# kcleal/pywfa

Measured on AMD Instinct MI355X. Metric: pairwise alignments/sec, higher is better.
Workload: dtype int16x2 offsets (reads <= 512 bp), int32 results; 1 GPU; C2: 10000000 x 150bp pairs/GPU, 2% error, gap-affine 0/4/6/2, end-to-end, scope=score, 2-bit reads resident in HBM; pairs_per_gpu=10000000, read_length=150, parallelism=pairs sharded over 1 GPU(s), no collective

## Files before the change

### pywfa_amd/csrc/wfa_lane.hpp

```cpp
#pragma once
#include "wfa_rtc_compat.hpp"
#include "wfa_common.hpp"
#include "wfa_hip.h"
#ifndef __HIPCC_RTC__
#include "wfa_rtc.hpp"
#endif

namespace wfa {

typedef short lane_s2 __attribute__((ext_vector_type(2)));
typedef unsigned short lane_u2 __attribute__((ext_vector_type(2)));

#define WFA_LANE_NULL16 (-16384)
#define WFA_LANE_NULL2 0xC000C000u
#ifndef WFA_LANE_DEBUG_COUNTERS
#define WFA_LANE_DEBUG_COUNTERS 0
#endif
#ifndef WFA_LANE_REGION_MARKS
#define WFA_LANE_REGION_MARKS 0
#endif
#if WFA_LANE_REGION_MARKS
#define WFA_LANE_MARK(name) asm volatile("; WFA_MARK " name ::: "memory")
#else
#define WFA_LANE_MARK(name)
#endif
#define WFA_LANE_COUNT(i) do { if (WFA_LANE_DEBUG_COUNTERS && !FULL && a.hist) { if (lane == 0) atomicAdd(reinterpret_cast<unsigned long long*>(a.hist) + (i), 1ull); } } while (0)

__device__ __forceinline__ uint32_t lane_ffbl(uint32_t x) {
  uint32_t r;
  asm("v_ffbl_b32 %0, %1" : "=v"(r) : "v"(x));
  return r;
}
__device__ __forceinline__ uint32_t pk_max(uint32_t a, uint32_t b) {
  lane_s2 r = __builtin_elementwise_max(__builtin_bit_cast(lane_s2, a), __builtin_bit_cast(lane_s2, b));
  return __builtin_bit_cast(uint32_t, r);
}
__device__ __forceinline__ uint32_t pk_min(uint32_t a, uint32_t b) {
  lane_s2 r = __builtin_elementwise_min(__builtin_bit_cast(lane_s2, a), __builtin_bit_cast(lane_s2, b));
  return __builtin_bit_cast(uint32_t, r);
}
__device__ __forceinline__ uint32_t pk_sub(uint32_t a, uint32_t b) {
  lane_s2 r = __builtin_bit_cast(lane_s2, a) - __builtin_bit_cast(lane_s2, b);
  return __builtin_bit_cast(uint32_t, r);
}
__device__ __forceinline__ uint32_t pk_add(uint32_t a, uint32_t b) {
  lane_s2 r = __builtin_bit_cast(lane_s2, a) + __builtin_bit_cast(lane_s2, b);
  return __builtin_bit_cast(uint32_t, r);
}
__device__ __forceinline__ uint32_t pk_clamp(uint32_t nm, uint32_t lim) {
#ifndef __HIPCC_RTC__
  uint32_t d, m, r;
  asm("v_pk_sub_i16 %0, %1, %2" : "=v"(d) : "v"(lim), "v"(nm));
  asm("v_pk_ashrrev_i16 %0, 15, %1 op_sel_hi:[0,1]" : "=v"(m) : "v"(d));
  asm("v_bfi_b32 %0, %1, %2, %3" : "=v"(r) : "v"(m), "s"(WFA_LANE_NULL2), "v"(nm));
  return r;
#else
  lane_s2 d = __builtin_bit_cast(lane_s2, lim) - __builtin_bit_cast(lane_s2, nm);
  d = d >> (short)15;
  const uint32_t m = __builtin_bit_cast(uint32_t, d);
  return (nm & ~m) | (WFA_LANE_NULL2 & m);
#endif
}

#ifndef WFA_LANE_WAVES_PER_EU
#define WFA_LANE_WAVES_PER_EU 0
#endif
#if WFA_LANE_WAVES_PER_EU > 0
#define WFA_LANE_OCCUPANCY __attribute__((amdgpu_waves_per_eu(WFA_LANE_WAVES_PER_EU, WFA_LANE_WAVES_PER_EU)))
#else
#define WFA_LANE_OCCUPANCY
#endif

template <int OE, int E>
struct LaneFull { static constexpr int NREC = 2 * (OE - E) + E * 17 + 1; };

template <int X, int OE, int E, bool FULL, bool HEUR = false, int LIN = 0, int NRP = 8>
__global__ void __launch_bounds__(64) WFA_LANE_OCCUPANCY
wfa_lane_kernel(const FastArgs a, const int slot_words_seq, const int refill_arg) {
  static_assert(!(FULL && HEUR), "the general form is score only");
  static_assert(NRP == 8 || (HEUR && NRP == 16) || (NRP == 4 && !FULL && !HEUR && LIN == 0),
                "the wider band exists in the general form only, the narrow one in the plain score-only form only");
  const int refill_min = refill_arg & 0xff;
  constexpr int NR = NRP, W = 2 * NR, H = NR;
  constexpr int DM = (X > OE) ? X : OE;
  constexpr int NEVER = 0x7fffffff;
  constexpr bool ENTRY = !FULL && !HEUR && LIN == 0;
  constexpr int K = ENTRY ? OE : 0, NCH = (OE + X - 1) / X;
  constexpr int NREC = LaneFull<OE, E>::NREC;
  extern __shared__ uint32_t lds[];
  const int slot_words = slot_words_seq;
  const int lane = threadIdx.x;
  uint32_t nwork = __builtin_amdgcn_readfirstlane(a.nwork_dev ? *a.nwork_dev : a.nwork);
  const bool dyn = !FULL && a.dyn_next != nullptr;
  bool exhausted = !dyn;
  uint32_t begin, end;
  auto grab = [&](uint32_t& b_, uint32_t& e_) -> bool {
    uint32_t nb = 0;
    if (lane == 0) nb = atomicAdd(a.dyn_next, a.dyn_chunk);
    nb = __builtin_amdgcn_readfirstlane(nb);
    if (nb >= nwork) return false;
    b_ = nb; e_ = (uint32_t)min((unsigned long long)nwork, (unsigned long long)nb + a.dyn_chunk);
    return true;
  };
  if (dyn) {
    if (!grab(begin, end)) return;
  } else {
    const uint32_t per = __builtin_amdgcn_readfirstlane((nwork + gridDim.x - 1) / gridDim.x);
    const unsigned long long begin64 = (unsigned long long)blockIdx.x * per;
    if (begin64 >= nwork) return;
    begin = (uint32_t)begin64;
    end = (uint32_t)min((unsigned long long)nwork, begin64 + per);
  }

  uint32_t pid0, pw0, ln0, pid1, pw1, ln1;
  auto load_window = [&](uint32_t wb, uint32_t& pid, uint32_t& pw, uint32_t& ln) {
    const unsigned long long idx = (unsigned long long)wb + lane;
    pid = 0u; pw = 0u; ln = 0u;
    if (idx < end) {
      pid = a.worklist ? a.worklist[a.work_begin + idx] : (uint32_t)(a.work_begin + idx);
      const WfaPairMeta m = a.meta[pid];
      pw = m.p_woff;
      ln = (m.plen > WFA_FAST_MAX_LEN || m.tlen > WFA_FAST_MAX_LEN) ? 0xffffffffu : ((uint32_t)m.plen | ((uint32_t)m.tlen << 16));
    }
  };
  uint32_t wbase = begin, next_i = begin;
  load_window(wbase, pid0, pw0, ln0);
  load_window(wbase + 64u, pid1, pw1, ln1);

  const int pbase = (4 + lane * slot_words) * 16;
  uint32_t cur[NR], lim[NR], Mh[DM][NR], Ih[E][NR], Dh[E][NR];
  uint32_t thr[HEUR ? NR : 1];
#pragma unroll
  for (int r = 0; r < NR; ++r) {
    cur[r] = WFA_LANE_NULL2; lim[r] = WFA_LANE_NULL2;
    if (HEUR) thr[r] = 0x3fff3fffu;
#pragma unroll
    for (int d = 0; d < DM; ++d) Mh[d][r] = WFA_LANE_NULL2;
#pragma unroll
    for (int d = 0; d < E; ++d) { Ih[d][r] = WFA_LANE_NULL2; Dh[d][r] = WFA_LANE_NULL2; }
  }
  int kb0 = pbase, tb = pbase;
  int jt = 0;
  uint32_t tend = 0xffffu;
  int s0 = 0, deadline = NEVER;
  uint32_t my_lb2 = 0, my_tl2 = 0;
  int steps_wait = 0, my_dinit = 0;
  bool edge_live = false;
  uint32_t mypid = 0;
  unsigned long long idle = ~0ull;
  int gstep = 0;
  uint32_t myslot = 0;
  uint2* const wave_codes = FULL ? a.codes + (unsigned long long)blockIdx.x * (unsigned long long)a.codes_cap * 64ull : nullptr;
  bool codes_full = false;
  __shared__ uint32_t rejq[128];
  int nrej = 0;
  auto rej_flush = [&]() {
    if (nrej == 0) return;
    uint32_t slot = 0;
    if (lane == 0) slot = atomicAdd(a.fb_count, (uint32_t)nrej);
    slot = __builtin_amdgcn_readfirstlane(slot);
    if (lane < nrej) a.fb_list[slot + lane] = rejq[lane];
    if (lane + 64 < nrej) a.fb_list[slot + 64 + lane] = rejq[64 + lane];
    nrej = 0;
  };

  while (true) {
    WFA_LANE_MARK("looptop_begin");
    const int nidle = __builtin_popcountll(idle);
    if (!exhausted && next_i >= end && (nidle >= refill_min || idle == ~0ull)) {
      if (grab(begin, end)) { wbase = begin; next_i = begin; load_window(wbase, pid0, pw0, ln0); load_window(wbase + 64u, pid1, pw1, ln1); }
      else exhausted = true;
    }
    if (next_i < end && (nidle >= refill_min || idle == ~0ull)) {
      WFA_LANE_MARK("refill_begin");
      WFA_LANE_COUNT(1);
      const bool is_idle = __builtin_amdgcn_inverse_ballot_w64(idle);
      const uint32_t rank = __builtin_amdgcn_mbcnt_hi((uint32_t)(idle >> 32), __builtin_amdgcn_mbcnt_lo((uint32_t)idle, 0u));
      const uint32_t navail = end - next_i;
      const bool take = is_idle && rank < navail;
      const uint32_t src = next_i + rank - wbase;
      const int sl = (int)(src & 63u);
      const uint32_t a_pid = __shfl(pid0, sl, 64), a_pw = __shfl(pw0, sl, 64), a_ln = __shfl(ln0, sl, 64);
      const uint32_t b_pid = __shfl(pid1, sl, 64), b_pw = __shfl(pw1, sl, 64), b_ln = __shfl(ln1, sl, 64);
      const bool hi_w = src >= 64u;
      const uint32_t n_pid = hi_w ? b_pid : a_pid, n_pw = hi_w ? b_pw : a_pw, n_ln = hi_w ? b_ln : a_ln;
      const int pl = (int)(n_ln & 0xffffu), tl = (int)(n_ln >> 16);
      const int nwp = (pl + 15) >> 4, ntot = nwp + ((tl + 15) >> 4);
      const int ak = tl - pl;
      const int pbf_ = (HEUR && a.ef) ? a.pbf : 0, tbf_ = (HEUR && a.ef) ? a.tbf : 0;
      const int dlo = min(-pbf_, ak), dhi = max(tbf_, ak);
      const bool bad = n_ln == 0xffffffffu || ntot + 1 > slot_words_seq ||
                       (HEUR ? (dhi - dlo > 2 * H - 3) : (ak < 1 - 2 * H || ak > 2 * H - 1));
      const unsigned long long tmask = __ballot(take);
      {
        unsigned long long lm = __ballot(take && !bad);
        while (lm) {
          const int L = __builtin_ctzll(lm);
          lm &= lm - 1ull;
          const uint32_t pw = __builtin_amdgcn_readlane(n_pw, L);
          const int nt = __builtin_amdgcn_readlane(ntot, L);
          if (lane < nt) __builtin_amdgcn_global_load_lds(a.words + pw + lane, &lds[4 + L * slot_words], 4, 0, 0);
        }
      }
      if (take) {
        const int c = bad ? 0 : (HEUR ? ((dlo + dhi + 1) >> 1) : ((ak + 1) >> 1));
        const int k0 = c - H;
        mypid = n_pid; s0 = gstep - K;
        if (FULL) myslot = next_i + rank;
        kb0 = pbase - k0; tb = pbase + nwp * 16;
        jt = bad ? 0 : ak - k0;
        tend = bad ? 0xffffu : (uint32_t)tl;
        deadline = bad ? gstep - 1
                       : HEUR ? gstep + 4 * (pl + tl) + 64
                       : s0 + min(2 * (OE - E) + E * (2 * c + 2 * H - ak), 2 * (OE - E) + E * (2 * H + 2 - 2 * c + ak))
                               - (FULL ? 1 : 0);
        const int j0 = -k0;
        const uint32_t lb2 = ((uint32_t)(pl + k0) & 0xffffu) | ((uint32_t)(pl + k0 + 1) << 16);
        const uint32_t tl2 = (uint32_t)tl | ((uint32_t)tl << 16);
        const int j0r = bad ? -1 : (j0 >> 1);
        const uint32_t c0 = (j0 & 1) ? ((uint32_t)WFA_LANE_NULL16 & 0xffffu) : (WFA_LANE_NULL2 & 0xffff0000u);
        if (HEUR) { my_lb2 = lb2; my_tl2 = tl2; steps_wait = a.steps_between; my_dinit = max(pl, tl); }
#pragma unroll
        for (int r = 0; r < NR; ++r) {
          lim[r] = bad ? WFA_LANE_NULL2 : pk_min(tl2, pk_add(lb2, (uint32_t)(2 * r) * 0x00010001u));
          cur[r] = (!ENTRY && j0r == r) ? c0 : WFA_LANE_NULL2;
          if (HEUR) {
            uint32_t c2 = 0, t2 = 0;
#pragma unroll
            for (int q = 0; q < 2; ++q) {
              const int k = k0 + 2 * r + q;
              int w0v = (k == 0) ? 0 : WFA_LANE_NULL16;
              if (a.ef && k >= -pbf_ && k <= tbf_) w0v = max(k, 0);
              int th = (k == ak) ? tl : 0x3fff;
              if (a.ef) th = min(max(tl, pl + k - a.pef), max(pl + k, tl - a.tef));
              if (bad) { w0v = WFA_LANE_NULL16; th = 0x3fff; }
              th = max(0, min(th, 0x3fff));
              c2 |= ((uint32_t)w0v & 0xffffu) << (16 * q);
              t2 |= ((uint32_t)th & 0xffffu) << (16 * q);
            }
            cur[r] = c2; thr[r] = t2;
          }
#pragma unroll
          for (int d = 0; d < DM; ++d) Mh[d][r] = WFA_LANE_NULL2;
#pragma unroll
          for (int d = 0; d < E; ++d) { Ih[d][r] = WFA_LANE_NULL2; Dh[d][r] = WFA_LANE_NULL2; }
        }
      }
      const uint32_t ntake = min((uint32_t)nidle, navail);
      next_i += ntake;
      idle &= ~tmask;
      __builtin_amdgcn_s_waitcnt(0x0F70);
      asm volatile("" ::: "memory");
      if (next_i - wbase >= 64u) {
        pid0 = pid1; pw0 = pw1; ln0 = ln1; wbase += 64u;
        load_window(wbase + 64u, pid1, pw1, ln1);
      }
      if constexpr (ENTRY) {
        const bool go = take && !bad;
        if (__any(go)) {
          WFA_LANE_MARK("entry_begin");
          WFA_LANE_COUNT(8);
          int ch[NCH];
#pragma unroll
          for (int i = 0; i < NCH; ++i) ch[i] = WFA_LANE_NULL16;
          const int etb = go ? tb : pbase;
          int ci = 0, ex = 0, lf = go ? min(pl, tl) : 0, fin_i = -1;
          bool act = go;
          do {
            WFA_LANE_MARK("entryround_begin");
            WFA_LANE_COUNT(9);
            const int v = ex + pbase, h = ex + etb;
            const uint32_t pa = ((uint32_t)v >> 2) & ~3u, ta = ((uint32_t)h >> 2) & ~3u;
            const uint32_t* pp = reinterpret_cast<const uint32_t*>(reinterpret_cast<const char*>(lds) + pa);
            const uint32_t* tp = reinterpret_cast<const uint32_t*>(reinterpret_cast<const char*>(lds) + ta);
            const uint32_t p0 = pp[0], p1 = pp[1], p2 = pp[2], t0 = tp[0], t1 = tp[1], t2 = tp[2];
            const uint32_t xl = __builtin_amdgcn_alignbit(p1, p0, (uint32_t)v << 1) ^ __builtin_amdgcn_alignbit(t1, t0, (uint32_t)h << 1);
            const uint32_t xh = __builtin_amdgcn_alignbit(p2, p1, (uint32_t)v << 1) ^ __builtin_amdgcn_alignbit(t2, t1, (uint32_t)h << 1);
            const uint32_t fb = min(lane_ffbl(xl), lane_ffbl(xh) | 32u);
            const int m = min((int)(fb >> 1), min(32, lf));
            ex += m; lf -= m;
            const bool stop = act && !((m == 32) && (lf > 0));
#pragma unroll
            for (int i = 0; i < NCH; ++i) ch[i] = (stop && ci == i) ? ex : ch[i];
            fin_i = (stop && ak == 0 && ex == tl) ? ci : fin_i;
            ci += stop ? 1 : 0;
            const bool on = stop && ci < NCH && lf > 0;
            act = stop ? on : act;
            ex += on ? 1 : 0; lf -= on ? 1 : 0;
            WFA_LANE_MARK("entryround_end");
          } while (__any(act));
          const bool fin = fin_i >= 0;
          if (fin) {
            a.score[mypid] = -__mul24(fin_i * X, a.g);
            a.status[mypid] = 0;
          }
          idle |= __ballot(fin);
          if (go) {
            auto place = [&](uint32_t (&dst)[NR], int slot, int val) {
              const int rr = fin ? -1 : (slot >> 1);
              const uint32_t w = (slot & 1) ? (((uint32_t)WFA_LANE_NULL16 & 0xffffu) | ((uint32_t)val << 16))
                                            : ((WFA_LANE_NULL2 & 0xffff0000u) | ((uint32_t)val & 0xffffu));
#pragma unroll
              for (int r = 0; r < NR; ++r) dst[r] = (rr == r) ? w : WFA_LANE_NULL2;
            };
            const int j0 = H - ((ak + 1) >> 1);
#pragma unroll
            for (int d = 0; d < DM; ++d) {
              const int sc = K - 1 - d;
              if (sc >= 0 && sc % X == 0) place(Mh[d], j0, ch[sc / X]);
            }
            place(Ih[0], j0 + 1, ch[0] + 1);
            place(Dh[0], j0 - 1, ch[0]);
            uint32_t mm[NR];
            if (K % X == 0) place(mm, j0, ch[NCH - 1] + 1);
#pragma unroll
            for (int r = 0; r < NR; ++r) {
              const uint32_t gap = pk_max(Ih[0][r], Dh[0][r]);
              cur[r] = pk_clamp((K % X == 0) ? pk_max(gap, mm[r]) : gap, lim[r]);
              if (fin) lim[r] = WFA_LANE_NULL2;
            }
            if (fin) { deadline = NEVER; jt = 0; tend = 0xffffu; }
          }
          WFA_LANE_MARK("entry_end");
        }
      }
      WFA_LANE_MARK("refill_end");
    } else if (idle == ~0ull && exhausted) {
      rej_flush();
      break;
    }

    int hot_j = -1, hot_x = 0, hot_left = 0;
#pragma unroll
    for (int r = 0; r < NR; ++r) {
      const uint32_t ua = pk_min(cur[r], pk_add(pk_sub(lim[r], cur[r]), 0xffffffffu));
      if (__any((ua & 0x80008000u) != 0x80008000u)) {
        WFA_LANE_MARK("probe_begin");
        WFA_LANE_COUNT(4);
        int off[2], left[2], x[2];
        bool valid[2], more[2];
#pragma unroll
        for (int q = 0; q < 2; ++q) {
          off[q] = q ? ((int)cur[r] >> 16) : (int)(short)(cur[r] & 0xffffu);
          const int lj = q ? ((int)lim[r] >> 16) : (int)(short)(lim[r] & 0xffffu);
          valid[q] = off[q] >= 0;
          left[q] = valid[q] ? lj - off[q] : 0;
        }
#pragma unroll
        for (int q = 0; q < 2; ++q) {
          const int j = 2 * r + q;
          x[q] = max(off[q], 0);
          const int v = x[q] + kb0 - j, h = x[q] + tb;
          const uint32_t pa = ((uint32_t)v >> 2) & ~3u, ta = ((uint32_t)h >> 2) & ~3u;
          const uint32_t* pp = reinterpret_cast<const uint32_t*>(reinterpret_cast<const char*>(lds) + pa);
          const uint32_t* tp = reinterpret_cast<const uint32_t*>(reinterpret_cast<const char*>(lds) + ta);
          const uint32_t p0 = pp[0], p1 = pp[1], t0 = tp[0], t1 = tp[1];
          const uint32_t xl = __builtin_amdgcn_alignbit(p1, p0, (uint32_t)v << 1) ^ __builtin_amdgcn_alignbit(t1, t0, (uint32_t)h << 1);
          const int m = min((int)(lane_ffbl(xl) >> 1), min(16, left[q]));
          x[q] += m; left[q] -= m;
          more[q] = (m == 16) && (left[q] > 0);
        }
#pragma unroll
        for (int q = 0; q < 2; ++q) {
          const int j = 2 * r + q;
          const bool park = more[q] && hot_j < 0;
          const bool now = more[q] && !park;
          hot_x = park ? x[q] : hot_x; hot_left = park ? left[q] : hot_left; hot_j = park ? j : hot_j;
          if (__any(now)) {
            WFA_LANE_MARK("nowfix_begin");
            WFA_LANE_COUNT(7);
            bool mo = now;
            int lf = mo ? left[q] : 0;
            int xx = x[q];
            do {
              WFA_LANE_MARK("now_begin");
              WFA_LANE_COUNT(5);
              const int v = xx + kb0 - j, h = xx + tb;
              const uint32_t pa = ((uint32_t)v >> 2) & ~3u, ta = ((uint32_t)h >> 2) & ~3u;
              const uint32_t* pp = reinterpret_cast<const uint32_t*>(reinterpret_cast<const char*>(lds) + pa);
              const uint32_t* tp = reinterpret_cast<const uint32_t*>(reinterpret_cast<const char*>(lds) + ta);
              const uint32_t p0 = pp[0], p1 = pp[1], p2 = pp[2], t0 = tp[0], t1 = tp[1], t2 = tp[2];
              const uint32_t xl = __builtin_amdgcn_alignbit(p1, p0, (uint32_t)v << 1) ^ __builtin_amdgcn_alignbit(t1, t0, (uint32_t)h << 1);
              const uint32_t xh = __builtin_amdgcn_alignbit(p2, p1, (uint32_t)v << 1) ^ __builtin_amdgcn_alignbit(t2, t1, (uint32_t)h << 1);
              const uint32_t fb = min(lane_ffbl(xl), lane_ffbl(xh) | 32u);
              const int m = min((int)(fb >> 1), min(32, lf));
              xx += m; lf -= m;
              mo = (m == 32) && (lf > 0);
              WFA_LANE_MARK("now_end");
            } while (__any(mo));
            x[q] = xx;
            WFA_LANE_MARK("nowfix_end");
          }
        }
        x[0] = valid[0] ? x[0] : off[0]; x[1] = valid[1] ? x[1] : off[1];
        cur[r] = ((uint32_t)x[0] & 0xffffu) | ((uint32_t)x[1] << 16);
        WFA_LANE_MARK("probe_end");
      }
    }
    if (__any(hot_j >= 0)) {
      bool mo = hot_j >= 0;
      int lf = mo ? hot_left : 0;
      const int kbj = kb0 - hot_j;
      WFA_LANE_COUNT(2);
      WFA_LANE_MARK("parkfix_begin");
      do {
        WFA_LANE_MARK("parked_begin");
        const int v = hot_x + kbj, h = hot_x + tb;
        const uint32_t pa = ((uint32_t)v >> 2) & ~3u, ta = ((uint32_t)h >> 2) & ~3u;
        const uint32_t* pp = reinterpret_cast<const uint32_t*>(reinterpret_cast<const char*>(lds) + pa);
        const uint32_t* tp = reinterpret_cast<const uint32_t*>(reinterpret_cast<const char*>(lds) + ta);
        const uint32_t p0 = pp[0], p1 = pp[1], p2 = pp[2], t0 = tp[0], t1 = tp[1], t2 = tp[2];
        const uint32_t xl = __builtin_amdgcn_alignbit(p1, p0, (uint32_t)v << 1) ^ __builtin_amdgcn_alignbit(t1, t0, (uint32_t)h << 1);
        const uint32_t xh = __builtin_amdgcn_alignbit(p2, p1, (uint32_t)v << 1) ^ __builtin_amdgcn_alignbit(t2, t1, (uint32_t)h << 1);
        const uint32_t fb = min(lane_ffbl(xl), lane_ffbl(xh) | 32u);
        const int m = min((int)(fb >> 1), min(32, lf));
        hot_x += m; lf -= m;
        mo = (m == 32) && (lf > 0);
        WFA_LANE_COUNT(3);
        WFA_LANE_MARK("parked_end");
      } while (__any(mo));
      const int hr = hot_j >> 1;
      const uint32_t hmask = (hot_j & 1) ? 0xffff0000u : 0x0000ffffu;
      const uint32_t hval = (hot_j & 1) ? ((uint32_t)hot_x << 16) : ((uint32_t)hot_x & 0xffffu);
#pragma unroll
      for (int r = 0; r < NR; ++r) {
        const uint32_t mk = (hr == r) ? hmask : 0u;
        cur[r] = (cur[r] & ~mk) | (hval & mk);
      }
      WFA_LANE_MARK("parkfix_end");
    }

    {
      uint32_t endv = 0;
      bool hit = false;
      if constexpr (HEUR) {
        uint32_t acc = 0;
#pragma unroll
        for (int r = 0; r < NR; ++r) acc |= ~pk_sub(cur[r], thr[r]);
        hit = (acc & 0x80008000u) != 0u;
      } else {
        uint32_t sel = cur[0];
#pragma unroll
        for (int r = 1; r < NR; ++r) sel = ((jt >> 1) == r) ? cur[r] : sel;
        endv = (jt & 1) ? (sel >> 16) : (sel & 0xffffu);
      }
      const unsigned long long active = ~idle;
      const unsigned long long bfin = __ballot(HEUR ? hit : (endv == tend)) & active;
      unsigned long long blimit = 0ull;
      if constexpr (HEUR) blimit = __ballot(a.max_steps != NEVER && __mul24(gstep - s0 + 1, a.g) >= a.max_steps) & active & ~bfin;
      const unsigned long long brej = __ballot(gstep > deadline || (HEUR && edge_live) || (FULL && codes_full)) & active & ~blimit;
      const unsigned long long bd = bfin | brej | blimit;
      if (bd) {
        WFA_LANE_MARK("bd_begin");
        WFA_LANE_COUNT(6);
        const unsigned long long ba = bfin & ~brej;
        if (__builtin_amdgcn_inverse_ballot_w64(ba)) {
          a.score[mypid] = -__mul24(gstep - s0, a.g);
          a.status[mypid] = 0;
          if (FULL) a.end_state[myslot] = make_int4((int)(blockIdx.x * (unsigned)a.codes_cap + (unsigned)gstep), lane | (jt << 8), gstep - s0, 1);
        }
        if (HEUR && __builtin_amdgcn_inverse_ballot_w64(blimit)) {
          a.score[mypid] = -a.max_steps;
          a.status[mypid] = WFA_STATUS_MAX_STEPS_REACHED;
        }
        if (brej) {
          if (__builtin_amdgcn_inverse_ballot_w64(brej)) {
            rejq[nrej + (int)__builtin_amdgcn_mbcnt_hi((uint32_t)(brej >> 32), __builtin_amdgcn_mbcnt_lo((uint32_t)brej, 0u))] = mypid;
            a.status[mypid] = WFA_INTERNAL_FALLBACK;
            if (FULL) a.end_state[myslot] = make_int4(0, 0, 0, 0);
          }
          nrej += __builtin_popcountll(brej);
          if (nrej >= 64) rej_flush();
        }
        if (__builtin_amdgcn_inverse_ballot_w64(bd)) {
#pragma unroll
          for (int r = 0; r < NR; ++r) { cur[r] = WFA_LANE_NULL2; lim[r] = WFA_LANE_NULL2; if (HEUR) thr[r] = 0x3fff3fffu; }
          deadline = NEVER; jt = 0; tend = 0xffffu; edge_live = false;
        }
        idle |= bd;
        WFA_LANE_MARK("bd_end");
        if (idle == ~0ull && next_i >= end && exhausted) { rej_flush(); break; }
      }
    }

    if constexpr (HEUR) {
      if (a.heur == 1) {
        auto mask16 = [&](const uint32_t (&x)[NR]) -> uint32_t {
          uint32_t lo16 = 0, hi16 = 0;
#pragma unroll
          for (int r = 0; r < NR; ++r) {
            const lane_u2 t = __builtin_bit_cast(lane_u2, x[r]) >> (unsigned short)15;
            const uint32_t w = (1u << (2 * (r & 7))) | (1u << (2 * (r & 7) + 17));
            if (r < 8) lo16 = __builtin_amdgcn_udot2(t, __builtin_bit_cast(lane_u2, w), lo16, false);
            else hi16 = __builtin_amdgcn_udot2(t, __builtin_bit_cast(lane_u2, w), hi16, false);
          }
          return ~(lo16 | (hi16 << 16)) & (NR == 16 ? 0xffffffffu : 0xffffu);
        };
        const uint32_t live = mask16(cur);
        if (live != 0u) --steps_wait;
        const int lo = (int)lane_ffbl(live), hi = 31 - (int)__builtin_clz(live | 1u);
        const bool consider = live != 0u && steps_wait <= 0 && (hi - lo + 1) >= a.min_wf_len && !__builtin_amdgcn_inverse_ballot_w64(idle);
        if (__any(consider)) {
          uint32_t d2[NR];
          uint32_t dm = 0x3fff3fffu;
#pragma unroll
          for (int r = 0; r < NR; ++r) {
            const uint32_t dl = pk_max(my_tl2, pk_add(my_lb2, (uint32_t)(2 * r) * 0x00010001u));
            const uint32_t dv = pk_sub(dl, cur[r]);
            const uint32_t dead = __builtin_bit_cast(uint32_t, __builtin_bit_cast(lane_s2, cur[r]) >> (short)15);
            d2[r] = (dv & ~dead) | (0x3fff3fffu & dead);
            dm = pk_min(dm, d2[r]);
          }
          const int dmin = min(my_dinit, min((int)(dm & 0xffffu), (int)(dm >> 16)));
          const uint32_t lim2 = (uint32_t)min(dmin + min(a.max_dist_thr, 0x3ffe), 0x3ffe) * 0x00010001u;
          uint32_t okx[NR];
#pragma unroll
          for (int r = 0; r < NR; ++r) okx[r] = pk_sub(lim2, d2[r]);
          const uint32_t okm = mask16(okx);
          const int lc = okm ? (int)lane_ffbl(okm) : 0x7fffffff, hc = okm ? 31 - (int)__builtin_clz(okm) : -0x7fffffff;
          const int akj = jt;
          int new_lo = lo, new_hi = hi;
          const int top_limit = min(akj, hi);
          if (top_limit > lo) new_lo = min(lc, top_limit);
          const int bottom_limit = max(akj, new_lo);
          if (bottom_limit < hi) new_hi = max(hc, bottom_limit);
          if (consider) steps_wait = a.steps_between;
          const bool cut = consider && (new_lo != lo || new_hi != hi);
          if (__any(cut)) {
            const uint32_t lo2 = (uint32_t)(cut ? new_lo : 0) * 0x00010001u, hi2 = (uint32_t)(cut ? new_hi : W - 1) * 0x00010001u;
#pragma unroll
            for (int r = 0; r < NR; ++r) {
              const uint32_t idx2 = (uint32_t)(2 * r) | ((uint32_t)(2 * r + 1) << 16);
              const uint32_t out = pk_sub(idx2, lo2) | pk_sub(hi2, idx2);
              const uint32_t km = ~__builtin_bit_cast(uint32_t, __builtin_bit_cast(lane_s2, out) >> (short)15);
              cur[r] = (cur[r] & km) | (WFA_LANE_NULL2 & ~km);
              Ih[0][r] = (Ih[0][r] & km) | (WFA_LANE_NULL2 & ~km);
              Dh[0][r] = (Dh[0][r] & km) | (WFA_LANE_NULL2 & ~km);
            }
          }
        }
      }
    }

    {
      uint32_t gi[NR], gd[NR];
#pragma unroll
      for (int r = 0; r < NR; ++r) {
        const uint32_t mo = (OE == 1) ? cur[r] : Mh[OE - 2][r];
        gi[r] = LIN ? mo : pk_max(mo, Ih[E - 1][r]);
        gd[r] = LIN ? mo : pk_max(mo, Dh[E - 1][r]);
      }
      uint32_t nm[NR], ni[NR], nd[NR];
      const uint32_t one2 = 0x00010001u;
      uint32_t cmp_i[FULL ? NR : 1], cmp_d[FULL ? NR : 1], cbyte[FULL ? NR : 1];
      if constexpr (FULL) {
#pragma unroll
        for (int r = 0; r < NR; ++r) {
          const uint32_t mo = (OE == 1) ? cur[r] : Mh[OE - 2][r];
          cmp_i[r] = LIN ? 0x80008000u : pk_sub(Ih[E - 1][r], mo);
          cmp_d[r] = LIN ? 0x80008000u : pk_sub(Dh[E - 1][r], mo);
        }
      }
#pragma unroll
      for (int r = 0; r < NR; ++r) {
        const uint32_t below = __builtin_amdgcn_alignbit(gi[r], (r > 0) ? gi[r - 1] : WFA_LANE_NULL2, 16);
        const uint32_t above = __builtin_amdgcn_alignbit((r < NR - 1) ? gd[r + 1] : WFA_LANE_NULL2, gd[r], 16);
        ni[r] = pk_add(below, one2);
        nd[r] = above;
        const uint32_t mx = (X == 1) ? cur[r] : Mh[X - 2][r];
        const uint32_t gap = pk_max(nd[r], ni[r]), x1 = (LIN == 2) ? WFA_LANE_NULL2 : pk_add(mx, one2);
        nm[r] = pk_clamp(pk_max(gap, x1), lim[r]);
        if constexpr (FULL) {
          const uint32_t ca = pk_sub(x1, gap), cb = pk_sub(nd[r], ni[r]);
          const uint32_t cc = __builtin_amdgcn_alignbit(cmp_i[r], (r > 0) ? cmp_i[r - 1] : 0u, 16);
          const uint32_t cd = __builtin_amdgcn_alignbit((r < NR - 1) ? cmp_d[r + 1] : 0u, cmp_d[r], 16);
          uint32_t t4 = (cc >> 2 & 0x20002000u) | (cd >> 3 & 0x10001000u);
          t4 = (cb >> 1 & 0x40004000u) | t4;
          t4 = (ca & 0x80008000u) | t4;
          cbyte[r] = ((t4 >> 12) & 0xFu) | ((t4 >> 24) & 0xF0u);
        }
      }
      if constexpr (FULL) {
        const uint32_t c0 = cbyte[0] | (cbyte[1] << 8) | (cbyte[2] << 16) | (cbyte[3] << 24);
        const uint32_t c1 = cbyte[4] | (cbyte[5] << 8) | (cbyte[6] << 16) | (cbyte[7] << 24);
        if (gstep + 1 < a.codes_cap) wave_codes[(unsigned)(gstep + 1) * 64u + (unsigned)lane] = make_uint2(c0, c1);
        else codes_full = true;
      }
#pragma unroll
      for (int r = 0; r < NR; ++r) {
#pragma unroll
        for (int d = DM - 1; d > 0; --d) Mh[d][r] = Mh[d - 1][r];
        Mh[0][r] = cur[r];
#pragma unroll
        for (int d = E - 1; d > 0; --d) { Ih[d][r] = Ih[d - 1][r]; Dh[d][r] = Dh[d - 1][r]; }
        Ih[0][r] = ni[r]; Dh[0][r] = nd[r];
        cur[r] = nm[r];
      }
      if constexpr (HEUR) {
        edge_live = (((nm[0] & ni[0] & nd[0]) & 0x00008000u) == 0u) || (((nm[NR - 1] & ni[NR - 1] & nd[NR - 1]) & 0x80000000u) == 0u);
      }
    }
    ++gstep;
  }
  if (WFA_LANE_DEBUG_COUNTERS && !FULL && a.hist) { if (lane == 0) atomicAdd(reinterpret_cast<unsigned long long*>(a.hist), (unsigned long long)gstep); }
}

#ifndef __HIPCC_RTC__
#define WFA_LANE_DECL(i, x, oe, e) \
  int launch_lane_s##i(unsigned grid, size_t smem, hipStream_t stream, const FastArgs& a, int slot_words, int refill_min, bool full, int heur, int nrp);
WFA_LANE_DECL(0, 2, 4, 1) WFA_LANE_DECL(1, 2, 3, 1) WFA_LANE_DECL(2, 4, 7, 1) WFA_LANE_DECL(3, 3, 5, 1)
WFA_LANE_DECL(4, 6, 8, 3) WFA_LANE_DECL(5, 5, 3, 3) WFA_LANE_DECL(6, 1, 2, 1)
#undef WFA_LANE_DECL

template <int X, int OE, int E>
inline int launch_lane_shape(unsigned grid, size_t smem, hipStream_t stream, const FastArgs& a, int slot_words, int refill_min, bool full, int heur, int nrp) {
  if (nrp == 4 && (full || heur)) return -1;
  if (nrp == 4) hipLaunchKernelGGL((wfa_lane_kernel<X, OE, E, false, false, 0, 4>), dim3(grid), dim3(64), smem, stream, a, slot_words, refill_min);
  else if (heur == 2) hipLaunchKernelGGL((wfa_lane_kernel<X, OE, E, false, true, 0, 16>), dim3(grid), dim3(64), smem, stream, a, slot_words, refill_min);
  else if (heur) hipLaunchKernelGGL((wfa_lane_kernel<X, OE, E, false, true>), dim3(grid), dim3(64), smem, stream, a, slot_words, refill_min);
  else if (full) hipLaunchKernelGGL((wfa_lane_kernel<X, OE, E, true>), dim3(grid), dim3(64), smem, stream, a, slot_words, refill_min);
  else hipLaunchKernelGGL((wfa_lane_kernel<X, OE, E, false>), dim3(grid), dim3(64), smem, stream, a, slot_words, refill_min);
  return hipGetLastError() == hipSuccess ? 0 : -1;
}

inline bool lane_heur_config(const WfaDevConfig& c, int ncomp) {
  return ncomp == 3 && c.match == 0 && c.wildcard < 0 && (c.heuristic == 0 || c.heuristic == 1);
}

inline int lane_slot_words(int max_len) {
  const int w = 2 * ((max_len + 15) >> 4) + 1;
  return w | 1;
}

inline int lane_full_records(int OE, int E) { return 2 * (OE - E) + E * 17 + 1; }
inline void lane_full_geometry(uint32_t nwork, int cu_count, int per_cu, int min_pairs, int OE, int E, long long* grid_out, int* cap_out) {
  if (min_pairs <= 0) min_pairs = 256;
  long long grid = (long long)cu_count * per_cu;
  const long long max_grid = ((long long)nwork + min_pairs - 1) / std::max(min_pairs, 64);
  if (grid > max_grid) grid = max_grid;
  if (grid < 1) grid = 1;
  const long long per = ((long long)nwork + grid - 1) / grid;
  const int nrec = lane_full_records(OE, E);
  *grid_out = grid;
  *cap_out = (int)(per * nrec / 32 + 2 * nrec + 8);
}

#define WFA_LANE_RUN_SLOT 32

inline int launch_lane_args(int shape_idx, int OE, int E, int cu_count, int per_cu, int refill_min, int max_len, hipStream_t stream, FastArgs a, bool full, int lds_pad_kb = 0, int min_pairs = 0, int heur = 0, int X = 0, int nrp = 8);

inline int launch_lane(int shape_idx, int g, int cu_count, int per_cu, int refill_min, int max_len, hipStream_t stream, const uint32_t* words,
                       const WfaPairMeta* meta, const uint32_t* worklist, const uint32_t* nwork_dev, uint32_t nwork,
                       int32_t* score, int32_t* status, uint32_t* fb_list, uint32_t* fb_count, int32_t* debug_counters = nullptr, int lds_pad_kb = 0,
                       int X = 0, int OE = 0, int E = 0, int min_pairs = 0, uint32_t* dyn_next = nullptr, uint32_t dyn_chunk = 0, int nrp = 8) {
  FastArgs a = FastArgs();
  a.dyn_next = dyn_chunk ? dyn_next : nullptr; a.dyn_chunk = dyn_chunk;
  a.words = words; a.meta = meta; a.worklist = worklist; a.nwork_dev = nwork_dev; a.nwork = nwork;
  a.score = score; a.status = status; a.fb_list = fb_list; a.fb_count = fb_count;
  a.g = g;
  a.hist = debug_counters; a.hist_stride = 0; a.end_state = nullptr; a.work_begin = 0;
  a.ef = a.pbf = a.pef = a.tbf = a.tef = 0; a.heur = 0; a.min_wf_len = a.max_dist_thr = a.steps_between = 0; a.max_steps = INT_MAX;
  return launch_lane_args(shape_idx, OE, E, cu_count, per_cu, refill_min, max_len, stream, a, false, lds_pad_kb, min_pairs, 0, X, nrp);
}

inline int launch_lane_args(int shape_idx, int OE, int E, int cu_count, int per_cu, int refill_min, int max_len, hipStream_t stream, FastArgs a, bool full, int lds_pad_kb, int min_pairs, int heur, int X, int nrp) {
  const uint32_t nwork = a.nwork;
  const uint32_t* nwork_dev = a.nwork_dev;
  const int slot_words = lane_slot_words(std::min(max_len, WFA_FAST_MAX_LEN));
  const size_t smem = ((size_t)64 * slot_words + 8) * sizeof(uint32_t) + (size_t)lds_pad_kb * 1024;
  long long grid = (long long)cu_count * per_cu;
  if (min_pairs <= 0) min_pairs = full ? 256 : (int)std::max<long long>(64, std::min<long long>(256, (long long)nwork / ((long long)cu_count * 16)));
  const long long max_grid = ((long long)nwork + min_pairs - 1) / std::max(min_pairs, 64);
  if (!nwork_dev && grid > max_grid) grid = max_grid;
  if (grid < 1) grid = 1;
  if (full && a.codes_cap <= 0) return -1;
  if (a.lin) shape_idx = WFA_SHAPE_RTC;
  if (nrp != 8 && nrp != 4) return -1;
  if (nrp == 4 && (shape_idx == WFA_SHAPE_RTC || full || heur)) return -1;
  switch (shape_idx) {
    case 0: return launch_lane_s0((unsigned)grid, smem, stream, a, slot_words, refill_min, full, heur, nrp);
    case 1: return launch_lane_s1((unsigned)grid, smem, stream, a, slot_words, refill_min, full, heur, nrp);
    case 2: return launch_lane_s2((unsigned)grid, smem, stream, a, slot_words, refill_min, full, heur, nrp);
    case 3: return launch_lane_s3((unsigned)grid, smem, stream, a, slot_words, refill_min, full, heur, nrp);
    case 4: return launch_lane_s4((unsigned)grid, smem, stream, a, slot_words, refill_min, full, heur, nrp);
    case 5: return launch_lane_s5((unsigned)grid, smem, stream, a, slot_words, refill_min, full, heur, nrp);
    case 6: return launch_lane_s6((unsigned)grid, smem, stream, a, slot_words, refill_min, full, heur, nrp);
    case WFA_SHAPE_RTC: {
      struct { FastArgs a; int slot_words; int refill_min; } args = {a, slot_words, refill_min};
      const std::string name = "wfa::wfa_lane_kernel<" + std::to_string(X) + ", " + std::to_string(OE) + ", " + std::to_string(E) + ", " +
                               rtc_bool(full && !heur) + ", " + rtc_bool(heur != 0) + (heur == 2 ? std::string(", 0, 16>") : a.lin ? ", " + std::to_string(a.lin) + ">" : std::string(">"));
      return rtc_launch("wfa_lane.hpp", name, (unsigned)grid, 64, smem, stream, &args, sizeof(args));
    }
    default: return -1;
  }
}

#endif

}
```

Before: 3.995 billion alignments/s.

## Precompute entry match chains per window from global memory and set occupancy hints

In the plain score-only form, the initial diagonal match-extension chains are now computed once per 64-pair window, straight from the 2-bit words in global memory, all lanes in parallel. The first chain end is packed into spare bits of the length word and the second goes to a small LDS array. This removes the serial per-refill LDS extend loop, and the window advance and waitcnt now run after the entry placement. The change also adds a default waves-per-EU hint computed from the register footprint, which can cause spills or limit occupancy.

```diff
diff --git a/pywfa_amd/csrc/wfa_lane.hpp b/pywfa_amd/csrc/wfa_lane.hpp
--- a/pywfa_amd/csrc/wfa_lane.hpp
+++ b/pywfa_amd/csrc/wfa_lane.hpp
@@ -68,7 +68,11 @@
 #if WFA_LANE_WAVES_PER_EU > 0
 #define WFA_LANE_OCCUPANCY __attribute__((amdgpu_waves_per_eu(WFA_LANE_WAVES_PER_EU, WFA_LANE_WAVES_PER_EU)))
 #else
-#define WFA_LANE_OCCUPANCY
+constexpr int lane_narrow_waves(int X, int OE, int E) {
+  const int R = ((X > OE) ? X : OE) + 2 * E + 2;
+  return R <= 6 ? 7 : R <= 8 ? 6 : R <= 11 ? 5 : 4;
+}
+#define WFA_LANE_OCCUPANCY __attribute__((amdgpu_waves_per_eu((NRP == 4) ? lane_narrow_waves(X, OE, E) : 1)))
 #endif
 
 template <int OE, int E>
@@ -86,6 +90,8 @@
   constexpr int NEVER = 0x7fffffff;
   constexpr bool ENTRY = !FULL && !HEUR && LIN == 0;
   constexpr int K = ENTRY ? OE : 0, NCH = (OE + X - 1) / X;
+  constexpr bool WINCH = ENTRY && NCH <= 2;
+  constexpr uint32_t LNM = WINCH ? 0x3ffu : 0xffffu;
   constexpr int NREC = LaneFull<OE, E>::NREC;
   extern __shared__ uint32_t lds[];
   const int slot_words = slot_words_seq;
@@ -113,6 +119,52 @@
   }
 
   uint32_t pid0, pw0, ln0, pid1, pw1, ln1;
+  __shared__ short wch[(WINCH && NCH == 2) ? 128 : 1];
+  auto window_chain = [&](uint32_t wb, uint32_t pw, uint32_t ln) -> uint32_t {
+    WFA_LANE_MARK("entry_begin");
+    WFA_LANE_COUNT(8);
+    const int pl = (int)(ln & 0xffffu), tl = (int)(ln >> 16);
+    const int nwp = (pl + 15) >> 4, ntot = nwp + ((tl + 15) >> 4), ak = tl - pl, L = min(pl, tl);
+    const bool elig = (unsigned long long)wb + lane < end &&
+                      !(ln == 0xffffffffu || ntot + 1 > slot_words_seq || ak < 1 - 2 * H || ak > 2 * H - 1);
+    bool act = elig;
+    const uint32_t* pp = a.words + pw;
+    int ch[NCH];
+#pragma unroll
+    for (int c = 0; c < NCH; ++c) ch[c] = WFA_LANE_NULL16;
+    int ci = 0;
+    const int imax = slot_words_seq >> 1;
+    int base = 0;
+#pragma nounroll
+    for (int i = 0; i < imax && __any(act); i += 2) {
+      WFA_LANE_MARK("entryround_begin");
+      WFA_LANE_COUNT(9);
+      uint32_t x0 = 0u, x1 = 0u;
+      if (act && base < L) x0 = pp[0] ^ pp[nwp];
+      if (act && base + 16 < L) x1 = pp[1] ^ pp[nwp + 1];
+      unsigned long long d = (unsigned long long)((x0 | (x0 >> 1)) & 0x55555555u) | ((unsigned long long)((x1 | (x1 >> 1)) & 0x55555555u) << 32);
+#pragma unroll
+      for (int c = 0; c < NCH; ++c) {
+        const int pos = d ? base + ((int)__builtin_ctzll(d) >> 1) : 0x7fff;
+        const bool hit = act && pos < L;
+#pragma unroll
+        for (int k = 0; k < NCH; ++k) ch[k] = (hit && ci == k) ? pos : ch[k];
+        ci += hit ? 1 : 0;
+        act = act && ci < NCH;
+        d &= d - 1ull;
+      }
+      const bool endc = act && base + 32 >= L;
+#pragma unroll
+      for (int k = 0; k < NCH; ++k) ch[k] = (endc && ci == k) ? L : ch[k];
+      act = act && !endc;
+      pp += 2; base += 32;
+      WFA_LANE_MARK("entryround_end");
+    }
+    if constexpr (NCH == 2) wch[64 + lane] = (short)ch[1];
+    WFA_LANE_MARK("entry_end");
+    const uint32_t c0 = (uint32_t)ch[0];
+    return elig ? (ln | ((c0 & 0x3fu) << 10) | ((c0 >> 6) << 26)) : ln;
+  };
   auto load_window = [&](uint32_t wb, uint32_t& pid, uint32_t& pw, uint32_t& ln) {
     const unsigned long long idx = (unsigned long long)wb + lane;
     pid = 0u; pw = 0u; ln = 0u;
@@ -124,8 +176,14 @@
     }
   };
   uint32_t wbase = begin, next_i = begin;
-  load_window(wbase, pid0, pw0, ln0);
-  load_window(wbase + 64u, pid1, pw1, ln1);
+  uint32_t wneed = 2u;
+  bool wmeta = false;
+  if constexpr (!WINCH) {
+    load_window(wbase, pid0, pw0, ln0);
+    load_window(wbase + 64u, pid1, pw1, ln1);
+  } else {
+    pid0 = pw0 = ln0 = pid1 = pw1 = ln1 = 0u;
+  }
 
   const int pbase = (4 + lane * slot_words) * 16;
   uint32_t cur[NR], lim[NR], Mh[DM][NR], Ih[E][NR], Dh[E][NR];
@@ -168,12 +226,28 @@
     WFA_LANE_MARK("looptop_begin");
     const int nidle = __builtin_popcountll(idle);
     if (!exhausted && next_i >= end && (nidle >= refill_min || idle == ~0ull)) {
-      if (grab(begin, end)) { wbase = begin; next_i = begin; load_window(wbase, pid0, pw0, ln0); load_window(wbase + 64u, pid1, pw1, ln1); }
-      else exhausted = true;
+      if (grab(begin, end)) {
+        wbase = begin; next_i = begin;
+        if constexpr (WINCH) { wneed = 2u; wmeta = false; }
+        else { load_window(wbase, pid0, pw0, ln0); load_window(wbase + 64u, pid1, pw1, ln1); }
+      } else exhausted = true;
     }
     if (next_i < end && (nidle >= refill_min || idle == ~0ull)) {
       WFA_LANE_MARK("refill_begin");
       WFA_LANE_COUNT(1);
+      if constexpr (WINCH) {
+#pragma nounroll
+        for (; wneed; --wneed) {
+          const uint32_t wb = wneed == 2u ? wbase : wbase + 64u;
+          if (!wmeta) load_window(wb, pid1, pw1, ln1);
+          wmeta = false;
+          ln1 = window_chain(wb, pw1, ln1);
+          if (wneed == 2u) {
+            pid0 = pid1; pw0 = pw1; ln0 = ln1;
+            if constexpr (NCH == 2) wch[lane] = wch[64 + lane];
+          }
+        }
+      }
       const bool is_idle = __builtin_amdgcn_inverse_ballot_w64(idle);
       const uint32_t rank = __builtin_amdgcn_mbcnt_hi((uint32_t)(idle >> 32), __builtin_amdgcn_mbcnt_lo((uint32_t)idle, 0u));
       const uint32_t navail = end - next_i;
@@ -184,7 +258,7 @@
       const uint32_t b_pid = __shfl(pid1, sl, 64), b_pw = __shfl(pw1, sl, 64), b_ln = __shfl(ln1, sl, 64);
       const bool hi_w = src >= 64u;
       const uint32_t n_pid = hi_w ? b_pid : a_pid, n_pw = hi_w ? b_pw : a_pw, n_ln = hi_w ? b_ln : a_ln;
-      const int pl = (int)(n_ln & 0xffffu), tl = (int)(n_ln >> 16);
+      const int pl = (int)(n_ln & LNM), tl = (int)((n_ln >> 16) & LNM);
       const int nwp = (pl + 15) >> 4, ntot = nwp + ((tl + 15) >> 4);
       const int ak = tl - pl;
       const int pbf_ = (HEUR && a.ef) ? a.pbf : 0, tbf_ = (HEUR && a.ef) ? a.tbf : 0;
@@ -249,47 +323,54 @@
       const uint32_t ntake = min((uint32_t)nidle, navail);
       next_i += ntake;
       idle &= ~tmask;
-      __builtin_amdgcn_s_waitcnt(0x0F70);
-      asm volatile("" ::: "memory");
-      if (next_i - wbase >= 64u) {
-        pid0 = pid1; pw0 = pw1; ln0 = ln1; wbase += 64u;
-        load_window(wbase + 64u, pid1, pw1, ln1);
+      if constexpr (!WINCH) {
+        __builtin_amdgcn_s_waitcnt(0x0F70);
+        asm volatile("" ::: "memory");
       }
       if constexpr (ENTRY) {
         const bool go = take && !bad;
         if (__any(go)) {
-          WFA_LANE_MARK("entry_begin");
-          WFA_LANE_COUNT(8);
           int ch[NCH];
-#pragma unroll
-          for (int i = 0; i < NCH; ++i) ch[i] = WFA_LANE_NULL16;
-          const int etb = go ? tb : pbase;
-          int ci = 0, ex = 0, lf = go ? min(pl, tl) : 0, fin_i = -1;
-          bool act = go;
-          do {
-            WFA_LANE_MARK("entryround_begin");
-            WFA_LANE_COUNT(9);
-            const int v = ex + pbase, h = ex + etb;
-            const uint32_t pa = ((uint32_t)v >> 2) & ~3u, ta = ((uint32_t)h >> 2) & ~3u;
-            const uint32_t* pp = reinterpret_cast<const uint32_t*>(reinterpret_cast<const char*>(lds) + pa);
-            const uint32_t* tp = reinterpret_cast<const uint32_t*>(reinterpret_cast<const char*>(lds) + ta);
-            const uint32_t p0 = pp[0], p1 = pp[1], p2 = pp[2], t0 = tp[0], t1 = tp[1], t2 = tp[2];
-            const uint32_t xl = __builtin_amdgcn_alignbit(p1, p0, (uint32_t)v << 1) ^ __builtin_amdgcn_alignbit(t1, t0, (uint32_t)h << 1);
-            const uint32_t xh = __builtin_amdgcn_alignbit(p2, p1, (uint32_t)v << 1) ^ __builtin_amdgcn_alignbit(t2, t1, (uint32_t)h << 1);
-            const uint32_t fb = min(lane_ffbl(xl), lane_ffbl(xh) | 32u);
-            const int m = min((int)(fb >> 1), min(32, lf));
-            ex += m; lf -= m;
-            const bool stop = act && !((m == 32) && (lf > 0));
-#pragma unroll
-            for (int i = 0; i < NCH; ++i) ch[i] = (stop && ci == i) ? ex : ch[i];
-            fin_i = (stop && ak == 0 && ex == tl) ? ci : fin_i;
-            ci += stop ? 1 : 0;
-            const bool on = stop && ci < NCH && lf > 0;
-            act = stop ? on : act;
-            ex += on ? 1 : 0; lf -= on ? 1 : 0;
-            WFA_LANE_MARK("entryround_end");
-          } while (__any(act));
-          const bool fin = fin_i >= 0;
+          int fin_i = -1;
+          if constexpr (WINCH) {
+            ch[0] = (int)(((n_ln >> 10) & 0x3fu) | (((n_ln >> 26) & 0xfu) << 6));
+            if constexpr (NCH == 2) ch[1] = (int)wch[src];
+#pragma unroll
+            for (int i = 0; i < NCH; ++i) fin_i = (ak == 0 && ch[i] == tl) ? i : fin_i;
+          } else {
+            WFA_LANE_MARK("entry_begin");
+            WFA_LANE_COUNT(8);
+#pragma unroll
+            for (int i = 0; i < NCH; ++i) ch[i] = WFA_LANE_NULL16;
+            const int etb = go ? tb : pbase;
+            int ci = 0, ex = 0, lf = go ? min(pl, tl) : 0;
+            bool act = go;
+            do {
+              WFA_LANE_MARK("entryround_begin");
+              WFA_LANE_COUNT(9);
+              const int v = ex + pbase, h = ex + etb;
+              const uint32_t pa = ((uint32_t)v >> 2) & ~3u, ta = ((uint32_t)h >> 2) & ~3u;
+              const uint32_t* pp = reinterpret_cast<const uint32_t*>(reinterpret_cast<const char*>(lds) + pa);
+              const uint32_t* tp = reinterpret_cast<const uint32_t*>(reinterpret_cast<const char*>(lds) + ta);
+              const uint32_t p0 = pp[0], p1 = pp[1], p2 = pp[2], t0 = tp[0], t1 = tp[1], t2 = tp[2];
+              const uint32_t xl = __builtin_amdgcn_alignbit(p1, p0, (uint32_t)v << 1) ^ __builtin_amdgcn_alignbit(t1, t0, (uint32_t)h << 1);
+              const uint32_t xh = __builtin_amdgcn_alignbit(p2, p1, (uint32_t)v << 1) ^ __builtin_amdgcn_alignbit(t2, t1, (uint32_t)h << 1);
+              const uint32_t fb = min(lane_ffbl(xl), lane_ffbl(xh) | 32u);
+              const int m = min((int)(fb >> 1), min(32, lf));
+              ex += m; lf -= m;
+              const bool stop = act && !((m == 32) && (lf > 0));
+#pragma unroll
+              for (int i = 0; i < NCH; ++i) ch[i] = (stop && ci == i) ? ex : ch[i];
+              fin_i = (stop && ak == 0 && ex == tl) ? ci : fin_i;
+              ci += stop ? 1 : 0;
+              const bool on = stop && ci < NCH && lf > 0;
+              act = stop ? on : act;
+              ex += on ? 1 : 0; lf -= on ? 1 : 0;
+              WFA_LANE_MARK("entryround_end");
+            } while (__any(act));
+            WFA_LANE_MARK("entry_end");
+          }
+          const bool fin = go && fin_i >= 0;
           if (fin) {
             a.score[mypid] = -__mul24(fin_i * X, a.g);
             a.status[mypid] = 0;
@@ -321,8 +402,19 @@
             }
             if (fin) { deadline = NEVER; jt = 0; tend = 0xffffu; }
           }
-          WFA_LANE_MARK("entry_end");
-        }
+        }
+      }
+      if constexpr (WINCH) {
+        __builtin_amdgcn_s_waitcnt(0x0F70);
+        asm volatile("" ::: "memory");
+      }
+      if (next_i - wbase >= 64u) {
+        pid0 = pid1; pw0 = pw1; ln0 = ln1; wbase += 64u;
+        if constexpr (WINCH) {
+          if constexpr (NCH == 2) wch[lane] = wch[64 + lane];
+          wneed = 1u; wmeta = true;
+        }
+        load_window(wbase + 64u, pid1, pw1, ln1);
       }
       WFA_LANE_MARK("refill_end");
     } else if (idle == ~0ull && exhausted) {
```

After: 4.260 billion alignments/s, median of 6. 6.7% higher.
